# chenzpstar/Multi-Modal-Image-Fusion

Measured on AMD Instinct MI355X. Metric: image-pairs/sec at 256x256, PFNet train step, higher is better.
Workload: dtype bf16; 1 GPU; PFNetv1 train step (fwd + SSIM/pixel/grad losses + bwd + clip + Adam), 256x256 synthetic IR/visible pairs, batch 32 per GPU, bf16 feature maps / fp32 accumulate, random-init weights (seed 0); global_batch=32, parallelism=single

## Files before the change

### multi-modal-image-fusion_amd/csrc/conv_mfma.hip

```cpp
#include "common.hpp"
#include "conv_route.hpp"
#include "wgrad_reduce.hpp"
#define MMIF_STORE_GRAN(p, v) (*reinterpret_cast<uint4*>(p) = (v))
#include <stdlib.h>

namespace mmif {

typedef __attribute__((ext_vector_type(8))) __bf16 bf16x8;
typedef __attribute__((ext_vector_type(4))) __bf16 bf16x4;
typedef __attribute__((ext_vector_type(4))) short s16x4;
typedef __attribute__((ext_vector_type(4))) float f32x4;
#define LDS_PTR(T, p) ((__attribute__((address_space(3))) T*)(p))

constexpr int DT_ROWS_C = DT_ROWS;
__host__ __device__ constexpr int plane_granules(int ks) { return ks == 3 ? 336 : 256; }

__host__ __device__ inline int visit_tap(int i, int ks) { return ks == 3 ? (i % 3) * 3 + i / 3 : i; }

static size_t packed_bytes(int n_out, int n_in, int ks) {
    const int ncb = (n_in + 7) / 8, kk = ks * ks;
    const size_t m16p = (size_t)n_mblocks(n_out) * pick_mf(n_out) * 16;
    size_t kg = 0;
    for (int c0 = 0; c0 < ncb; c0 += CHUNK_CB) {
        const int n = ncb - c0 < CHUNK_CB ? ncb - c0 : CHUNK_CB;
        kg += (size_t)((kk * n + 3) / 4) * 4;
    }
    return kg * m16p * 16;
}

__global__ void pack_weights_kernel(const float* __restrict__ w, int cout, int cin, int ks, int dgrad, int mf,
                                    int m16p, bf16_t* __restrict__ dst, long long total) {
    const int kk = ks * ks;
    const int n_out = dgrad ? cin : cout, n_in = dgrad ? cout : cin;
    const int ncb = (n_in + 7) / 8;
    for (long long idx = (long long)blockIdx.x * blockDim.x + threadIdx.x; idx < total; idx += (long long)gridDim.x * blockDim.x) {
        const int e = idx & 7;
        const long long row = idx >> 3;
        const int oc = (int)(row % m16p);
        long long kgp = row / m16p;
        int c0 = 0, n = 0, kg = 0;
        for (c0 = 0; c0 < ncb; c0 += CHUNK_CB) {
            n = ncb - c0 < CHUNK_CB ? ncb - c0 : CHUNK_CB;
            const int pad = ((kk * n + 3) / 4) * 4;
            if (kgp < pad) { kg = (int)kgp; break; }
            kgp -= pad;
        }
        float val = 0.f;
        if (kg < kk * n) {
            const int tap = kg / n, cb = kg % n;
            const int u = tap / ks, v = tap % ks;
            const int ic = (c0 + cb) * 8 + e;
            if (oc < n_out && ic < n_in) {
                if (dgrad) val = w[(((long long)ic * cin + oc) * ks + (ks - 1 - u)) * ks + (ks - 1 - v)];
                else val = w[(((long long)oc * cin + ic) * ks + u) * ks + v];
            }
        }
        dst[idx] = f32_to_bf16(val);
    }
    (void)mf;
}

constexpr int PACK_MAX_IMAGES = 64;
struct PackImage { const float* w; bf16_t* dst; long long total; int cout, cin, ks, dgrad, m16p; };
struct PackTable { PackImage im[PACK_MAX_IMAGES]; };

__device__ inline void pack_gran(const PackImage& J, long long row) {
    const int ks = J.ks, kk = ks * ks, cin = J.cin, m16p = J.m16p;
    const int n_out = J.dgrad ? cin : J.cout, n_in = J.dgrad ? J.cout : cin;
    const int ncb = (n_in + 7) / 8;
    const int oc = (int)(row % m16p);
    long long kgp = row / m16p;
    int c0 = 0, n = 0, kg = 0;
    for (c0 = 0; c0 < ncb; c0 += CHUNK_CB) {
        n = ncb - c0 < CHUNK_CB ? ncb - c0 : CHUNK_CB;
        const int pad = ((kk * n + 3) / 4) * 4;
        if (kgp < pad) { kg = (int)kgp; break; }
        kgp -= pad;
    }
    float val[8];
#pragma unroll
    for (int e = 0; e < 8; ++e) val[e] = 0.f;
    if (kg < kk * n && oc < n_out) {
        const int tap = kg / n, cb = kg % n;
        const int u = tap / ks, v = tap % ks;
        const int ic0 = (c0 + cb) * 8;
#pragma unroll
        for (int e = 0; e < 8; ++e) {
            const int ic = ic0 + e;
            if (ic < n_in) {
                if (J.dgrad) val[e] = J.w[(((long long)ic * cin + oc) * ks + (ks - 1 - u)) * ks + (ks - 1 - v)];
                else val[e] = J.w[(((long long)oc * cin + ic) * ks + u) * ks + v];
            }
        }
    }
    *reinterpret_cast<uint4*>(J.dst + row * 8) = make_uint4(pack_bf16x2(val[0], val[1]), pack_bf16x2(val[2], val[3]), pack_bf16x2(val[4], val[5]), pack_bf16x2(val[6], val[7]));
}

__global__ void pack_weights_multi_kernel(PackTable tab) {
    const PackImage& J = tab.im[blockIdx.y];
    const long long rows = J.total >> 3;
    for (long long row = (long long)blockIdx.x * blockDim.x + threadIdx.x; row < rows; row += (long long)gridDim.x * blockDim.x)
        pack_gran(J, row);
}

__device__ inline uint4 ld_gran(const TV& t, int in_, int c, int ys, int xs) {
    return *reinterpret_cast<const uint4*>(t.base + t.gidx(in_, c, ys, xs) * 16);
}
__device__ inline uint4 load_in_reflect(const TV& t, int in_, int c, int y, int x) {
    y = min(max(reflect_idx(y, t.h), 0), t.h - 1);
    x = min(max(reflect_idx(x, t.w), 0), t.w - 1);
    return ld_gran(t, in_, c, y, x);
}
__device__ inline uint4 load_in_gradfold(const TV& t, int in_, int c, int y, int x) {
    if (y < 0 || y >= t.h || x < 0 || x >= t.w) return make_uint4(0, 0, 0, 0);
    if (t.halo == 0 || t.folded) return ld_gran(t, in_, c, y + t.halo, x + t.halo);
    const bool by = (y == 1) || (y == t.h - 2), bx = (x == 1) || (x == t.w - 2);
    if (!by && !bx) return ld_gran(t, in_, c, y + 1, x + 1);
    float v[8];
    load_grad_fold<bf16_t>(t, in_, c, y, x, v);
    return make_uint4(pack_bf16x2(v[0], v[1]), pack_bf16x2(v[2], v[3]), pack_bf16x2(v[4], v[5]), pack_bf16x2(v[6], v[7]));
}

struct DupOut {
    TV out, mask;
    int frag;
};

template <int MF, bool DGRAD, bool LM = false, bool DUP = false>
__device__ inline void conv_epilogue(const f32x4 (&acc)[MF][4], const TV& tout, const TV& tmask, const float* s_bias, int mb, int in_,
                                     int oxs, int oys0, int g, int relu, unsigned long long mask_bits, unsigned long long accum_bits,
                                     int xlim, int ylim,
                                     const unsigned char* lmask = nullptr, int lrow0 = 0, int lcol = 0,
                                     const TV* told = nullptr ,
                                     const DupOut* dup = nullptr ) {
    if (oxs >= xlim) return;
    const unsigned row_bytes = (unsigned)tout.ws * 16u;
    const unsigned pix_off = (unsigned)(oys0 * tout.ws + oxs) * 16u;
    uint4 oldv[(DGRAD && !DUP) ? MF : 1][2], xmv[(DGRAD && !LM && !DUP) ? MF : 1][2];
    unsigned lbits[(DGRAD && LM) ? MF : 1][2];
    if (DGRAD && LM) {
#pragma unroll
        for (int m = 0; m < MF; ++m)
#pragma unroll
            for (int p2 = 0; p2 < 2; ++p2) lbits[LM ? m : 0][p2] = lmask[((2 * m + (g >> 1)) * DT_ROWS_C + lrow0 + 2 * p2) * MT + lcol];
    }
    if (DGRAD && !DUP) {
        const unsigned mpix_off = (unsigned)min(max(reflect_idx(oxs - tout.halo, tmask.w), 0), tmask.w - 1) * 16u;
#pragma unroll
        for (int m = 0; m < MF; ++m) {
            const int ocb = (mb * MF + m) * 2 + (g >> 1);
            const bool blk_ok = ocb < tout.cb;
            const char* oplane = tout.base + ((long long)in_ * tout.img + (long long)(tout.cb_off + min(ocb, tout.cb - 1)) * tout.plane) * 16 + pix_off;
            if (told != nullptr)
                oplane = told->base + ((long long)in_ * told->img + (long long)(told->cb_off + min(ocb, told->cb - 1)) * told->plane) * 16 +
// ... 240 lines not shown
        } else {
            const bool inside = y >= 0 && y < tin.h && x >= 0 && x < tin.w;
            const bool border = tin.halo && !tin.folded && ((y == 1) || (y == tin.h - 2) || (x == 1) || (x == tin.w - 2));
            mode = !inside ? 0 : (border ? 2 : 1);
            ioff[i] = (unsigned)((min(max(y, 0), tin.h - 1) + tin.halo) * tin.ws + min(max(x, 0), tin.w - 1) + tin.halo) * 16u;
        }
        idesc[i] = (cb * PL + p) | (cb << 16) | (mode << 20);
        ioff[i] += (unsigned)min(cb, CHUNK_CB - 1) * (unsigned)(tin.plane * 16);
    }
    const char* in_img = tin.base + ((long long)in_ * tin.img + (long long)tin.cb_off * tin.plane) * 16;
    const bool fold_tile = DGRAD && tin.halo && !tin.folded &&
                           ((iy0 <= 1 && 1 < iy0 + TP) || (iy0 <= tin.h - 2 && tin.h - 2 < iy0 + TP) ||
                            (ix0 <= 1 && 1 < ix0 + TP) || (ix0 <= tin.w - 2 && tin.w - 2 < ix0 + TP));

    f32x4 acc[MF][4];
#pragma unroll
    for (int m = 0; m < MF; ++m)
#pragma unroll
        for (int n = 0; n < 4; ++n) acc[m][n] = (f32x4){0.f, 0.f, 0.f, 0.f};

    const int ncb_tot = tin.cb;
    const char* in_lane = reinterpret_cast<const char*>(s_in) + ((wave * 4) * TP + j) * 16;
    const char* w_lane = reinterpret_cast<const char*>(s_w) + j * 16;

    constexpr bool WREG = (256 % (MF * 16)) == 0;
    constexpr int NWO = WREG ? 1 : NW;
    unsigned woff[NWO];
#pragma unroll
    for (int i = 0; i < NWO; ++i) {
        const int e = tid + 256 * i;
        woff[i] = (unsigned)((e / (MF * 16)) * m16p + mb * MF * 16 + e % (MF * 16)) * 16u;
    }
    const unsigned wstride = (unsigned)(256 / (MF * 16)) * (unsigned)m16p * 16u;
    uint4 rin[NIN], rw[NW];
    auto issue_load = [&](int i, int c0, long long wchunk_off) {
        const int ncb = min(CHUNK_CB, ncb_tot - c0);
        if (i < NIN) {
            const int cb = (idesc[i] >> 16) & 15, mode = idesc[i] >> 20;
            const char* chunk = in_img + (long long)c0 * tin.plane * 16;
            const uint4 v = *reinterpret_cast<const uint4*>(chunk + (cb < ncb ? ioff[i] : ioff[0]));
            rin[i] = (cb < ncb && mode >= 1) ? v : make_uint4(0, 0, 0, 0);
        } else if (i < NIN + NW) {
            const int nkgp = (KK * ncb + 3) / 4 * 4;
            const char* wchunk = reinterpret_cast<const char*>(wpk + wchunk_off);
            const int e = tid + 256 * (i - NIN);
            uint4 v = make_uint4(0, 0, 0, 0);
            if (e / (MF * 16) < nkgp) {
                if (WREG) v = *reinterpret_cast<const uint4*>(wchunk + (long long)(i - NIN) * wstride + woff[0]);
                else v = *reinterpret_cast<const uint4*>(wchunk + woff[WREG ? 0 : i - NIN]);
            }
            rw[i - NIN] = v;
        }
    };
    auto prefetch = [&](int c0, long long wchunk_off) {
#pragma unroll
        for (int i = 0; i < NIN + NW; ++i) issue_load(i, c0, wchunk_off);
    };
    if (!DGRAD && tid < MF * 16) {
        const int oc = mb * MF * 16 + tid;
        s_bias[tid] = (bias != nullptr && oc < n_out) ? bias[oc] : 0.f;
    }

    long long wchunk_off = 0;
    TRACE_STAMP();
    prefetch(0, 0);
    TRACE_STAMP();
    for (int c0 = 0; c0 < ncb_tot; c0 += CHUNK_CB) {
        const int ncb = min(CHUNK_CB, ncb_tot - c0);
        const int nkg = KK * ncb, nkgp = (nkg + 3) / 4 * 4;
        __syncthreads();
        TRACE_STAMP();
#pragma unroll
        for (int i = 0; i < NIN; ++i)
            if (((idesc[i] >> 16) & 15) < ncb) s_in[idesc[i] & 0xffff] = rin[i];
        if (DGRAD && fold_tile) {
#pragma unroll 1
            for (int e = tid; e < ncb * TP * TP; e += 256) {
                const int cb = e / (TP * TP), p = e % (TP * TP);
                const int y = iy0 + p / TP, x = ix0 + p % TP;
                const bool inside = y >= 0 && y < tin.h && x >= 0 && x < tin.w;
                if (inside && ((y == 1) || (y == tin.h - 2) || (x == 1) || (x == tin.w - 2)))
                    s_in[cb * PL + p] = load_in_gradfold(tin, in_, c0 + cb, y, x);
            }
        }
#pragma unroll
        for (int i = 0; i < NW; ++i) {
            const int e = tid + 256 * i;
            if (e < nkgp * MF * 16) s_w[e] = rw[i];
        }
        if (tid < nkgp) {
            int tap = 0, cb = 0, plane = tid;
            if (tid < nkg) { tap = visit_tap(tid / ncb, KS); cb = tid % ncb; plane = tap * ncb + cb; }
            s_tab[tid] = make_int2((cb * PL + (tap / KS) * TP + (tap % KS)) * 16, plane * MF * 256);
        }
        TRACE_STAMP();
        __syncthreads();
        TRACE_STAMP();
        wchunk_off += (long long)nkgp * m16p;
        const bool have_next = c0 + CHUNK_CB < ncb_tot;
        const int nsteps = nkgp >> 2;
        if (have_next) prefetch(c0 + CHUNK_CB, wchunk_off);
        int2 off = s_tab[g];
        int2 nxt = s_tab[min(4, nkgp - 4) + g];
        bf16x8 b[4];
#pragma unroll
        for (int n = 0; n < 4; ++n) b[n] = *reinterpret_cast<const bf16x8*>(in_lane + off.x + n * TP * 16);
        for (int s = 0; s < nsteps; ++s) {
            const int2 nxt2 = s_tab[min(4 * (s + 2), nkgp - 4) + g];
            bf16x8 a[MF], bn[4];
#pragma unroll
            for (int m = 0; m < MF; ++m) a[m] = *reinterpret_cast<const bf16x8*>(w_lane + off.y + m * 256);
#pragma unroll
            for (int n = 0; n < 4; ++n) bn[n] = *reinterpret_cast<const bf16x8*>(in_lane + nxt.x + n * TP * 16);
#pragma unroll
            for (int m = 0; m < MF; ++m)
#pragma unroll
                for (int n = 0; n < 4; ++n) acc[m][n] = __builtin_amdgcn_mfma_f32_16x16x32_bf16(a[m], b[n], acc[m][n], 0, 0, 0);
#pragma unroll
            for (int n = 0; n < 4; ++n) b[n] = bn[n];
            off = nxt;
            nxt = nxt2;
        }
        TRACE_STAMP();
    }

    conv_epilogue<MF, DGRAD>(acc, tout, tmask, s_bias, mb, in_, tile_x * MT + j, tile_y * MT + wave * 4 + (g & 1), g, relu, mask_bits,
                             accum_bits, tout.ws, tout.hs);
    TRACE_STAMP();
    if (tr != nullptr) tr[63] = tr_n;
#undef TRACE_STAMP
}

constexpr int DTP_Y = DT_ROWS + 2, DTP_X = MT + 2;
constexpr int DPL = 624;
constexpr int DIN_PIECES = CHUNK_CB * DPL / 64;
constexpr int DW_PIECES = 36;
constexpr int D_PIECES = DIN_PIECES + DW_PIECES;
constexpr int DBUF_BYTES = CHUNK_CB * DPL * 16 + DW_PIECES * 64 * 16;
static_assert(CHUNK_CB * DPL % 64 == 0, "input planes must be whole DMA pieces");

#define MMIF_GPTR(p) ((const __attribute__((address_space(1))) void*)(p))
#define MMIF_LPTR(p) ((__attribute__((address_space(3))) void*)(p))

struct DItem { int mb, in_, tile_y, tile_x; };

template <int N> struct IC { static constexpr int value = N; };

template <int MF, int NBUF = (MF == 3 ? 1 : 2)>
__device__ inline void dgrad_fold_steps(f32x4 (&acc)[MF][4], const char* in_c, const char* w_c, int ncb, int pitch, int g, int j, int yl,
                                        int xl, int hs, int ws) {
    const int nb = hs - 4 - yl;
    const int jl = 1 - xl, jr = ws - 4 - xl;
    const bool has_t = yl == 0, has_b = nb >= 0 && nb < 4, has_l = jl >= 0, has_r = jr >= 0 && jr < MT;
    if (!(has_t || has_b || has_l || has_r)) return;
    const bf16x8 zero8 = __builtin_bit_cast(bf16x8, make_uint4(0, 0, 0, 0));
    const bool kz = g >= ncb;
    auto ldb = [&](int brow, int bcol, int jsel) {
        bf16x8 b = *reinterpret_cast<const bf16x8*>(in_c + (brow * pitch + bcol) * 16);
        if (kz || (jsel >= 0 && j != jsel)) b = zero8;
        return b;
    };
    auto lda = [&](int tap, int m) { return *reinterpret_cast<const bf16x8*>(w_c + tap * ncb * (MF * 256) + m * 256); };
    auto at_row = [&](int n, auto&& f) {
        if (n == 0) f(IC<0>()); else if (n == 1) f(IC<1>()); else if (n == 2) f(IC<2>()); else f(IC<3>());
    };
    auto row_steps = [&](auto nc, int tap0, int brow) {
        constexpr int n = decltype(nc)::value;
        bf16x8 b[3], a[3][MF];
#pragma unroll
        for (int v = 0; v < 3; ++v) {
            b[v] = ldb(brow, v, -1);
#pragma unroll
            for (int m = 0; m < MF; ++m) a[v][m] = lda(tap0 + v, m);
        }
#pragma unroll
        for (int v = 0; v < 3; ++v)
#pragma unroll
            for (int m = 0; m < MF; ++m) acc[m][n] = __builtin_amdgcn_mfma_f32_16x16x32_bf16(a[v][m], b[v], acc[m][n], 0, 0, 0);
    };
    auto col_steps = [&](int vcol, int bcol, int jsel) {
        constexpr int NB = NBUF;
        bf16x8 a[NB][MF], b[NB][4];
        auto fetch = [&](int u, int slot) {
#pragma unroll
            for (int m = 0; m < MF; ++m) a[slot][m] = lda(3 * u + vcol, m);
#pragma unroll
            for (int n = 0; n < 4; ++n) b[slot][n] = ldb(n + u, bcol, jsel);
        };
        if (NB == 2) fetch(0, 0);
#pragma unroll
        for (int u = 0; u < 3; ++u) {
            if (NB == 1) fetch(u, 0);
            else if (u + 1 < 3) fetch(u + 1, (u + 1) & 1);
#pragma unroll
            for (int m = 0; m < MF; ++m)
#pragma unroll
                for (int n = 0; n < 4; ++n)
                    acc[m][n] = __builtin_amdgcn_mfma_f32_16x16x32_bf16(a[u & (NB - 1)][m], b[u & (NB - 1)][n], acc[m][n], 0, 0, 0);
        }
    };
    auto corner = [&](auto nc, int tap, int brow, int bcol, int jsel) {
        constexpr int n = decltype(nc)::value;
        const bf16x8 b = ldb(brow, bcol, jsel);
#pragma unroll
        for (int m = 0; m < MF; ++m) acc[m][n] = __builtin_amdgcn_mfma_f32_16x16x32_bf16(lda(tap, m), b, acc[m][n], 0, 0, 0);
    };
    if (has_t) {
        row_steps(IC<1>(), 6, 1);
        if (has_l) corner(IC<1>(), 8, 1, 0, jl);
        if (has_r) corner(IC<1>(), 6, 1, 2, jr);
    }
    if (has_b) {
        at_row(nb, [&](auto nc) {
            constexpr int n = decltype(nc)::value;
            row_steps(nc, 0, n + 2);
            if (has_l) corner(nc, 2, n + 2, 0, jl);
            if (has_r) corner(nc, 0, n + 2, 2, jr);
        });
    }
    if (has_l) col_steps(2, 0, jl);
    if (has_r) col_steps(0, 2, jr);
}

constexpr int D_CONS = 8;
constexpr int D_LOAD = 4;
constexpr int DL_IN_ITERS = (DIN_PIECES + D_LOAD - 1) / D_LOAD;

constexpr int SIGN_XOFF = 15;
struct SignMap {
    unsigned char* p;
    int cb, hs, pitch;
};
static inline int sign_pitch(int w) { return (cdiv(w, MT) + 2) * MT; }

template <bool DIAG> struct DiagArgs {};
template <> struct DiagArgs<true> {
    long long* trace;
    int abl;
};
template <bool DGRAD, int LMASK, bool DUP = false, bool DIAG = false>
__global__ __launch_bounds__((D_CONS + D_LOAD) * 64, 3) void conv_dma_kernel(TV tin, TV tout, TV tmask, const uint4* __restrict__ wpk,
                                                                              const float* __restrict__ bias, int n_out, int m16p, int relu,
                                                                              unsigned long long mask_bits, unsigned long long accum_bits,
                                                                              int tiles_x, int tiles_y, int nmb, int org, SignMap sgn, DupOut dup,
                                                                              DiagArgs<DIAG> diag) {
    constexpr int MF = 4;
    long long* trace = nullptr;
    int abl = 0;
    if constexpr (DIAG) { trace = diag.trace; abl = diag.abl; }
    __shared__ __attribute__((aligned(16))) char s_buf[2 * DBUF_BYTES];
    __shared__ int2 s_tab[2][DW_PIECES];
    __shared__ __attribute__((aligned(16))) float s_bias[3][MF * 16];
    __shared__ __attribute__((aligned(16))) int4 s_item[3];
    __shared__ __attribute__((aligned(16))) unsigned char s_mask[LMASK ? 2 : 1][LMASK ? 8 * DT_ROWS * MT : 16];

    const int tid = threadIdx.x, lane = tid & 63;
    const int wave = __builtin_amdgcn_readfirstlane(tid >> 6);
    const int j = lane & 15, g = lane >> 4;
    int tr_n = 0;
    long long* tr = (trace != nullptr && blockIdx.x < 128 && lane == 0 && wave < D_CONS) ? trace + ((long long)blockIdx.x * 8 + wave) * 64 : nullptr;
#define DTRACE() do { if (tr != nullptr && tr_n < 62 && !(abl & 256)) tr[tr_n++] = (long long)__builtin_amdgcn_s_memtime(); } while (0)
#define DTRACE_TOP(q) do { if (tr != nullptr && tr_n < 62 && (!(abl & 256) || (q) % 3 == 0)) tr[tr_n++] = (long long)__builtin_amdgcn_s_memtime(); } while (0)
    if (tr != nullptr && tr_n < 62) tr[tr_n++] = (long long)__builtin_amdgcn_s_memtime();
    const int tpi = tiles_x * tiles_y;
    const int nitems = tpi * tout.n * nmb;
    int first, stride, count;
    {
        const int G = gridDim.x, b = blockIdx.x;
        if ((G & 7) == 0) {
            const int xcd = b & 7, slot = b >> 3, nsl = G >> 3;
            const int q8 = nitems >> 3, r8 = nitems & 7;
            const int band0 = xcd < r8 ? xcd * (q8 + 1) : r8 * (q8 + 1) + (xcd - r8) * q8;
            const int blen = q8 + (xcd < r8 ? 1 : 0);
            first = band0 + slot;
            stride = nsl;
            count = blen > slot ? (blen - slot + nsl - 1) / nsl : 0;
        } else {
            first = b;
            stride = G;
            count = b < nitems ? (nitems - b + G - 1) / G : 0;
        }
    }
    if (count == 0) return;
    auto decode = [&](int lin) {
        DItem it;
        const unsigned ul = (unsigned)lin, unmb = (unsigned)nmb, utpi = (unsigned)tpi, utx = (unsigned)tiles_x;
        const unsigned tl = ul / unmb;
        it.mb = (int)(ul - tl * unmb);
        const unsigned uin = tl / utpi, trem = tl - uin * utpi;
        const unsigned ty = trem / utx;
        unsigned txx = trem - ty * utx;
        if (org) txx = (txx + ty + uin) % utx;
        it.in_ = (int)uin;
        it.tile_y = (int)ty;
        it.tile_x = (int)txx;
        return it;
    };
    const int ncb_tot = tin.cb;
    const int nch = (ncb_tot + CHUNK_CB - 1) / CHUNK_CB;
    const int ncb_last = ncb_tot - (nch - 1) * CHUNK_CB;
    const int total_q = count * nch;
    if (tid < DW_PIECES) {
        const int kg = tid;
        int tap = 0, cb = 0, plane = kg;
        if (kg < 9 * ncb_last) { tap = visit_tap(kg / ncb_last, 3); cb = kg % ncb_last; plane = tap * ncb_last + cb; }
        s_tab[1][kg] = make_int2((cb * DPL + (tap / 3) * DTP_X + (tap % 3)) * 16, plane * MF * 256);
    }
// ... 42 lines not shown
            char* dst_in = s_buf + buf * DBUF_BYTES + lw * 1024;
            char* dst_w = s_buf + buf * DBUF_BYTES + CHUNK_CB * DPL * 16 + kgf * 1024;
            const char* src_in = tin.base + ((long long)itm.in_ * tin.img + (long long)(tin.cb_off + c * CHUNK_CB) * tin.plane) * 16;
            const char* src_w = reinterpret_cast<const char*>(wpk) + ((long long)c * DW_PIECES * m16p + itm.mb * MF * 16) * 16;
            auto pieces = [&](auto full_c) {
                constexpr bool FULL = decltype(full_c)::value != 0;
                if (!skip_in) {
#pragma unroll
                    for (int i = 0; i < DL_IN_ITERS; ++i) {
                        if (i == DL_IN_ITERS - 1 && lw + D_LOAD * i >= DIN_PIECES) break;
                        unsigned off = d_off[i];
                        if (!FULL) {
                            const unsigned cb = (d_cb >> (2 * i)) & 3u;
                            off -= (cb - min(cb, (unsigned)(ncb - 1))) * plane_bytes;
                        }
                        __builtin_amdgcn_global_load_lds(MMIF_GPTR(src_in + off), MMIF_LPTR(dst_in + i * (D_LOAD * 1024)), 16, 0, 0);
                    }
                }
                if (!skip_w) {
                    unsigned woff = w_off0;
                    const int wlim = nkgp - kgf;
#pragma unroll
                    for (int k = 0; k < DW_PIECES / D_LOAD; ++k) {
                        if (FULL || D_LOAD * k < wlim)
                            __builtin_amdgcn_global_load_lds(MMIF_GPTR(src_w + woff), MMIF_LPTR(dst_w + k * (D_LOAD * 1024)), 16, 0, 0);
                        woff += D_LOAD * wstep;
                    }
                }
            };
            if (ncb == CHUNK_CB) pieces(IC<1>());
            else pieces(IC<0>());
        };
        auto load_bias = [&](const DItem& itm, int slot) {
            static_assert(MF * 16 == 64, "the M-block's bias is one wave's worth");
            if (!DGRAD && lw == 0) {
                const int oc = itm.mb * MF * 16 + lane;
                s_bias[slot][lane] = (bias != nullptr && oc < n_out) ? bias[oc] : 0.f;
            }
        };
        uint4 mreg[LMASK == 1 ? 16 : 1];
        bool mpend = false;
        int mpar = 0;
        auto issue_mask = [&](const DItem& itm) {
            const int t = tid - D_CONS * 64;
            if (LMASK == 2) {
                const int cbl = t >> 5, row = t & 31;
                const int ocb = itm.mb * 8 + cbl;
                const bool need = ocb < tout.cb && ((mask_bits >> ocb) & 1ull);
                const int ys = min(org + itm.tile_y * DT_ROWS + row, sgn.hs - 1), xs = org + itm.tile_x * MT;
                mreg[0] = make_uint4(0xffffffffu, 0xffffffffu, 0xffffffffu, 0xffffffffu);
                if (need) mreg[0] = *reinterpret_cast<const uint4*>(sgn.p + (((long long)itm.in_ * sgn.cb + min(ocb, sgn.cb - 1)) * sgn.hs + ys) * sgn.pitch + xs + SIGN_XOFF);
                return;
            }
#pragma unroll
            for (int cbl = 0; cbl < 8; ++cbl) {
                const int ocb = itm.mb * 8 + cbl;
                const bool need = ocb < tout.cb && ((mask_bits >> ocb) & 1ull);
#pragma unroll
                for (int k = 0; k < 2; ++k) {
                    const int p = t + 256 * k, row = p >> 4, col = p & 15;
                    const int oys = org + itm.tile_y * DT_ROWS + row, oxs = org + itm.tile_x * MT + col;
                    const int y = min(max(reflect_idx(oys - tout.halo, tmask.h), 0), tmask.h - 1);
                    const int x = min(max(reflect_idx(oxs - tout.halo, tmask.w), 0), tmask.w - 1);
                    if (need) mreg[LMASK == 1 ? 2 * cbl + k : 0] = *reinterpret_cast<const uint4*>(tmask.base + tmask.gidx(itm.in_, min(ocb, tmask.cb - 1), y, x) * 16);
                }
            }
        };
        auto park_mask = [&](const DItem& itm, int par) {
            const int t = tid - D_CONS * 64;
            if (LMASK == 2) {
                *reinterpret_cast<uint4*>(&s_mask[LMASK ? par : 0][LMASK ? t * MT : 0]) = mreg[0];
                return;
            }
#pragma unroll
            for (int cbl = 0; cbl < 8; ++cbl) {
                const int ocb = itm.mb * 8 + cbl;
                const bool need = ocb < tout.cb && ((mask_bits >> ocb) & 1ull);
                if (!need) continue;
#pragma unroll
                for (int k = 0; k < 2; ++k) {
                    const uint4 v = mreg[LMASK == 1 ? 2 * cbl + k : 0];
                    const uint32_t wv[4] = {v.x, v.y, v.z, v.w};
                    unsigned bits = 0;
#pragma unroll
                    for (int i = 0; i < 4; ++i) {
                        bits |= ((short)(wv[i] & 0xffffu) > 0 ? 1u : 0u) << (2 * i);
                        bits |= ((short)(wv[i] >> 16) > 0 ? 1u : 0u) << (2 * i + 1);
                    }
                    s_mask[LMASK ? par : 0][LMASK ? cbl * (DT_ROWS * MT) + t + 256 * k : 0] = (unsigned char)bits;
                }
            }
        };
        auto publish = [&](const DItem& itm, int slot) {
            if (lw == 0) {
                s_item[slot] = make_int4(itm.mb, itm.in_, itm.tile_y, itm.tile_x);
                __asm__ volatile("s_waitcnt lgkmcnt(0)" ::: "memory");
            }
        };
        DItem cur = decode(first), mitem = cur;
        publish(cur, 0);
        make_desc(cur);
        load_bias(cur, 0);
        issue_dma(cur, 0, 0);
        int c = 0, item_i = 0;
        if (LMASK && nch == 2) { issue_mask(cur); mitem = cur; mpar = 0; mpend = true; }
        for (int q = 0; q < total_q; ++q) {
            __builtin_amdgcn_s_waitcnt(0x0f70);
            __builtin_amdgcn_s_barrier();
            if (LMASK && mpend) {
                park_mask(mitem, mpar);
                __asm__ volatile("s_waitcnt lgkmcnt(0)" ::: "memory");
                mpend = false;
            }
            if (++c == nch) {
                c = 0;
                ++item_i;
                if (q + 1 < total_q) {
                    cur = decode(first + item_i * stride);
                    publish(cur, item_i % 3);
                    make_desc(cur);
                    load_bias(cur, item_i % 3);
                }
            }
            if (q + 1 < total_q && !(abl & 1)) issue_dma(cur, c, (q & 1) ^ 1, item_i);
            if (LMASK && q + 1 < total_q && c == nch - 2) { issue_mask(cur); mitem = cur; mpar = item_i & 1; mpend = true; }
        }
        return;
    }

    f32x4 acc[MF][4];
#define DMA_EPILOGUE(itm, slot, par)                                                                                                          \
    do {                                                                                                                                      \
        const int oxs_ = org + (itm).tile_x * MT + j, oys0_ = org + (itm).tile_y * DT_ROWS + wave * 4 + (g & 1);                              \
        if constexpr (!DGRAD) {                                                                                                               \
            conv_epilogue_packed<MF, false>(acc, tout, s_bias[slot], (itm).mb, (itm).in_, org + (itm).tile_x * MT,                            \
                                            org + (itm).tile_y * DT_ROWS + wave * 4, wave * 4, relu, mask_bits, tout.ws - org, tout.hs - org,  \
                                            nullptr, tr, &tr_n);                                                                                     \
        } else if constexpr (LMASK != 0) {                                                                                                    \
            if (accum_bits == 0)                                                                                                              \
                conv_epilogue_packed<MF, true>(acc, tout, s_bias[slot], (itm).mb, (itm).in_, org + (itm).tile_x * MT,                         \
                                               org + (itm).tile_y * DT_ROWS + wave * 4, wave * 4, relu, mask_bits, tout.ws - org,             \
                                               tout.hs - org, s_mask[LMASK ? (par) : 0]);                                                     \
            else                                                                                                                              \
                conv_epilogue<MF, true, true>(acc, tout, tmask, s_bias[slot], (itm).mb, (itm).in_, oxs_, oys0_, g, relu, mask_bits,           \
                                              accum_bits, tout.ws - org, tout.hs - org, s_mask[LMASK ? (par) : 0], wave * 4 + (g & 1), j);    \
        } else {                                                                                                                              \
            conv_epilogue<MF, true, false, DUP>(acc, tout, tmask, s_bias[slot], (itm).mb, (itm).in_, oxs_, oys0_, g, relu, mask_bits,        \
                                                accum_bits, tout.ws - org, tout.hs - org, nullptr, wave * 4 + (g & 1), j, nullptr, &dup);     \
        }                                                                                                                                     \
    } while (0)
    DItem cur = {0, 0, 0, 0}, pend = cur;
    bool have_pend = false;
    int pend_slot = 0, pend_par = 0;
    int c = 0, item_i = 0;
    for (int q = 0; q < total_q; ++q) {
        const int buf = q & 1;
        DTRACE_TOP(q);
        __builtin_amdgcn_s_barrier();
        DTRACE();
        int lane_q;
        __asm__ volatile("v_mbcnt_lo_u32_b32 %0, -1, 0\n\tv_mbcnt_hi_u32_b32 %0, -1, %0" : "=v"(lane_q));
        const int j = lane_q & 15, g = lane_q >> 4;
        if (c == 0) {
            const int4 it4 = s_item[item_i % 3];
            cur.mb = __builtin_amdgcn_readfirstlane(it4.x);
            cur.in_ = __builtin_amdgcn_readfirstlane(it4.y);
            cur.tile_y = __builtin_amdgcn_readfirstlane(it4.z);
            cur.tile_x = __builtin_amdgcn_readfirstlane(it4.w);
        }
        if (have_pend) {
            __builtin_amdgcn_s_setprio(3);
            DMA_EPILOGUE(pend, pend_slot, pend_par);
            __builtin_amdgcn_s_setprio(0);
            have_pend = false;
        }
        DTRACE();
        const int ncb = min(CHUNK_CB, ncb_tot - c * CHUNK_CB);
        const char* in_lane = s_buf + buf * DBUF_BYTES + ((wave * 4) * DTP_X + j) * 16;
        const char* w_lane = s_buf + buf * DBUF_BYTES + CHUNK_CB * DPL * 16 + j * 16;
        const bool rows_live = !DGRAD || org + cur.tile_y * DT_ROWS + wave * 4 < tout.hs - org;
        if (c == 0) {
#pragma unroll
            for (int m = 0; m < MF; ++m)
#pragma unroll
                for (int n = 0; n < 4; ++n) acc[m][n] = (f32x4){0.f, 0.f, 0.f, 0.f};
        }
        if (!rows_live) {
        } else if (ncb == CHUNK_CB) {
            const char* in_g = in_lane + g * (DPL * 16);
            const char* w_g = w_lane + g * (MF * 256);
            bf16x8 a[2][MF], rows[8];
            auto ld_row = [&](int v, int r) { return *reinterpret_cast<const bf16x8*>(in_g + (r * DTP_X + v) * 16); };
            auto ld_a = [&](int t, int slot) {
                const int tap = (t % 3) * 3 + t / 3;
#pragma unroll
                for (int m = 0; m < MF; ++m) a[slot][m] = *reinterpret_cast<const bf16x8*>(w_g + tap * 4 * MF * 256 + m * 256);
            };
#pragma unroll
            for (int r = 0; r < 4; ++r) rows[r] = ld_row(0, r);
            ld_a(0, 0);
#pragma unroll
            for (int t = 0; t < 9; ++t) {
                const int v = t / 3, u = t % 3;
                int nreads = 0;
                if (t + 1 < 9) {
                    const int v1 = (t + 1) / 3, u1 = (t + 1) % 3;
                    if (u1 == 0) {
#pragma unroll
                        for (int r = 0; r < 4; ++r) rows[(6 * v1 + r) % 8] = ld_row(v1, r);
                        nreads += 4;
                    } else {
                        rows[(6 * v1 + 3 + u1) % 8] = ld_row(v1, 3 + u1);
                        nreads += 1;
                    }
                    ld_a(t + 1, (t + 1) & 1);
                    nreads += MF;
                }
#pragma unroll
                for (int m = 0; m < MF; ++m)
#pragma unroll
                    for (int n = 0; n < 4; ++n)
                        acc[m][n] = __builtin_amdgcn_mfma_f32_16x16x32_bf16(a[t & 1][m], rows[(6 * v + u + n) % 8], acc[m][n], 0, 0, 0);
                if (t + 1 < 9) {
#pragma unroll
                    for (int r = 0; r < 5; ++r) {
                        __builtin_amdgcn_sched_group_barrier(0x100, 1, 0);
                        __builtin_amdgcn_sched_group_barrier(0x008, 1, 0);
                    }
                    if ((t + 1) % 3 == 0) {
#pragma unroll
                        for (int r = 0; r < 3; ++r) {
                            __builtin_amdgcn_sched_group_barrier(0x100, 1, 0);
                            __builtin_amdgcn_sched_group_barrier(0x008, 1, 0);
                        }
                        __builtin_amdgcn_sched_group_barrier(0x008, 8, 0);
                    } else {
                        __builtin_amdgcn_sched_group_barrier(0x008, 11, 0);
                    }
                }
                (void)nreads;
            }
        } else {
            const int nkgp = (9 * ncb + 3) / 4 * 4, nsteps = nkgp >> 2;
            const int2* tab = s_tab[1];
            int2 off = tab[g];
            int2 nx = tab[min(4, nkgp - 4) + g];
            bf16x8 b[4];
#pragma unroll
            for (int n = 0; n < 4; ++n) b[n] = *reinterpret_cast<const bf16x8*>(in_lane + off.x + n * DTP_X * 16);
            for (int s2 = 0; s2 < nsteps; ++s2) {
                const int2 nx2 = tab[min(4 * (s2 + 2), nkgp - 4) + g];
                bf16x8 a[MF], bn[4];
#pragma unroll
                for (int m = 0; m < MF; ++m) a[m] = *reinterpret_cast<const bf16x8*>(w_lane + off.y + m * 256);
#pragma unroll
                for (int n = 0; n < 4; ++n) bn[n] = *reinterpret_cast<const bf16x8*>(in_lane + nx.x + n * DTP_X * 16);
#pragma unroll
                for (int m = 0; m < MF; ++m)
#pragma unroll
                    for (int n = 0; n < 4; ++n) acc[m][n] = __builtin_amdgcn_mfma_f32_16x16x32_bf16(a[m], b[n], acc[m][n], 0, 0, 0);
#pragma unroll
                for (int n = 0; n < 4; ++n) b[n] = bn[n];
                off = nx;
                nx = nx2;
            }
        }
        if (DGRAD && org && rows_live && !(abl & 4))
            dgrad_fold_steps<MF>(acc, in_lane + min(g, ncb - 1) * (DPL * 16), w_lane + min(g, ncb - 1) * (MF * 256), ncb, DTP_X, g, j,
                                 cur.tile_y * DT_ROWS + wave * 4, cur.tile_x * MT, tout.hs, tout.ws);
        DTRACE();
        if (++c == nch) {
            c = 0;
            if (wave < 4) {
                DMA_EPILOGUE(cur, item_i % 3, item_i & 1);
            } else {
                pend = cur;
                pend_slot = item_i % 3;
                pend_par = item_i & 1;
                have_pend = true;
            }
            ++item_i;
        }
        DTRACE();
    }
    if (tr != nullptr) { tr[63] = tr_n; tr[62] = (long long)__builtin_amdgcn_s_memtime(); }
#undef DTRACE
#undef DTRACE_TOP
    if (have_pend) DMA_EPILOGUE(pend, pend_slot, pend_par);
#undef DMA_EPILOGUE
}


__device__ inline void tn_wait_vmcnt(int n) {
    switch (n) {
        case 0: __builtin_amdgcn_s_waitcnt(0x0f70); break;
        case 1: __builtin_amdgcn_s_waitcnt(0x0f71); break;
        case 2: __builtin_amdgcn_s_waitcnt(0x0f72); break;
        case 3: __builtin_amdgcn_s_waitcnt(0x0f73); break;
        case 4: __builtin_amdgcn_s_waitcnt(0x0f74); break;
        case 5: __builtin_amdgcn_s_waitcnt(0x0f75); break;
        case 6: __builtin_amdgcn_s_waitcnt(0x0f76); break;
        case 7: __builtin_amdgcn_s_waitcnt(0x0f77); break;
        case 8: __builtin_amdgcn_s_waitcnt(0x0f78); break;
        case 9: __builtin_amdgcn_s_waitcnt(0x0f79); break;
        case 10: __builtin_amdgcn_s_waitcnt(0x0f7a); break;
        case 11: __builtin_amdgcn_s_waitcnt(0x0f7b); break;
        case 12: __builtin_amdgcn_s_waitcnt(0x0f7c); break;
        case 13: __builtin_amdgcn_s_waitcnt(0x0f7d); break;
        case 14: __builtin_amdgcn_s_waitcnt(0x0f7e); break;
        case 15: __builtin_amdgcn_s_waitcnt(0x0f7f); break;
        default: __builtin_amdgcn_s_waitcnt(0x4f70); break;
    }
}
__device__ inline void tn_wait_counter(volatile unsigned* ctr, unsigned target) {
    const unsigned a = (unsigned)(size_t)ctr;
    for (int spin = 0; spin < (1 << 22); ++spin) {
        unsigned v;
        __asm__ volatile("ds_read_b32 %0, %1\n\ts_waitcnt lgkmcnt(0)" : "=v"(v) : "v"(a) : "memory");
        if (v >= target) break;
        __builtin_amdgcn_s_sleep(1);
    }
    __asm__ volatile("" ::: "memory");
}

template <int MF, bool DGRAD, int GROUPS = TN_GROUPS, int PL = TN_PL, int MAXP = 8, int RING = tn_ring_bytes(MF), bool TIGHT = false>
__global__ __launch_bounds__((4 * GROUPS + TN_LOAD) * 64, GROUPS == TN_GROUPS ? 4 : 3) void thin_conv_async_kernel(
    TV tin, TV tout, TV tmask, const uint4* __restrict__ wpk, const float* __restrict__ bias, int n_out, int relu,
    unsigned long long mask_bits, unsigned long long accum_bits, int tiles_x, int tiles_y, int ntiles, int org, TV told, int use_old) {
    constexpr int TP = MT + 2;
    constexpr int NCONS = 4 * GROUPS;
    __shared__ __attribute__((aligned(16))) char s_in[RING];
    __shared__ __attribute__((aligned(16))) uint4 s_w[TN_MAXKG * MF * 16];
    __shared__ int2 s_tab[2][36];
    __shared__ __attribute__((aligned(16))) float s_bias[MF * 16];
    __shared__ unsigned s_ready[TN_MAXSLOTS], s_done[TN_MAXSLOTS];
    const int tid = threadIdx.x, lane = tid & 63;
    const int wave = __builtin_amdgcn_readfirstlane(tid >> 6);
    const int j = lane & 15, g = lane >> 4;
    const int G = gridDim.x, b = blockIdx.x;
    const int tpi = tiles_x * tiles_y;
    const int ncb_tot = tin.cb;
    const int nch = (ncb_tot + CHUNK_CB - 1) / CHUNK_CB;
    const int nmine = b < ntiles ? (ntiles - b + G - 1) / G : 0;
    if (nmine == 0) return;
    auto tile_of = [&](int i, int& in_, int& tile_y, int& tile_x) {
        int lin = i;
        if ((G & 7) == 0) {
            const int q8 = ntiles >> 3, r8 = ntiles & 7, xcd = i & 7;
            lin = (xcd < r8 ? xcd * (q8 + 1) : r8 * (q8 + 1) + (xcd - r8) * q8) + (i >> 3);
        }
        in_ = lin / tpi;
        const int trem = lin - in_ * tpi;
        tile_y = trem / tiles_x;
        tile_x = trem - tile_y * tiles_x;
        if (org) tile_x = (tile_x + tile_y + in_) % tiles_x;
    };
    const int in_pieces = (ncb_tot * PL + 63) / 64;
    const int P = (in_pieces + TN_LOAD - 1) / TN_LOAD;
    const int slot_bytes = TIGHT ? in_pieces * 1024 : P * TN_LOAD * 1024;
    const int NS = min(TN_MAXSLOTS, RING / slot_bytes);
    const int D = min(2, NS - GROUPS);

    if (tid < 72) {
        const int c = tid / 36, kg = tid % 36;
        const int ncb = min(CHUNK_CB, ncb_tot - c * CHUNK_CB);
        if (ncb > 0) {
            int tap = 0, cb = 0, plane = kg;
            if (kg < 9 * ncb) { tap = visit_tap(kg / ncb, 3); cb = kg % ncb; plane = tap * ncb + cb; }
            s_tab[c][kg] = make_int2(((c * CHUNK_CB + cb) * PL + (tap / 3) * TP + (tap % 3)) * 16, (c * 36 + plane) * MF * 256);
        }
    }
    if (!DGRAD && tid < MF * 16) s_bias[tid] = (bias != nullptr && tid < n_out) ? bias[tid] : 0.f;
    if (tid < TN_MAXSLOTS) { s_ready[tid] = 0u; s_done[tid] = 0u; }
    if (wave >= NCONS) {
        int wbytes = 0;
        for (int c = 0; c < nch; ++c) wbytes += ((9 * min(CHUNK_CB, ncb_tot - c * CHUNK_CB) + 3) / 4 * 4) * MF * 256;
        const char* src = reinterpret_cast<const char*>(wpk) + lane * 16;
        char* dst = reinterpret_cast<char*>(s_w);
        for (int pz = wave - NCONS; pz * 1024 < wbytes; pz += TN_LOAD)
            __builtin_amdgcn_global_load_lds(MMIF_GPTR(src + (long long)pz * 1024), MMIF_LPTR(dst + pz * 1024), 16, 0, 0);
        __builtin_amdgcn_s_waitcnt(0x0f70);
    }
    __syncthreads();

    if (wave >= NCONS) {
        const int lw = wave - NCONS;
        unsigned geo[MAXP];
#pragma unroll
        for (int i = 0; i < MAXP; ++i) {
            const int slot = min(min(lw + TN_LOAD * i, in_pieces - 1) * 64 + lane, ncb_tot * PL - 1);
            const int pl = slot / PL, p = min(slot - pl * PL, TP * TP - 1);
            geo[i] = (unsigned)(pl << 16 | (p / TP) << 8 | (p % TP));
        }
        const unsigned plane_bytes = (unsigned)(tin.plane * 16);
        auto issue_tile = [&](int k) {
            int in_, ty0, tx0;
            tile_of(b + k * G, in_, ty0, tx0);
            const int iy0 = ty0 * MT - tout.halo - 1 + org, ix0 = tx0 * MT - tout.halo - 1 + org;
            const char* src = tin.base + ((long long)in_ * tin.img + (long long)tin.cb_off * tin.plane) * 16;
            char* dst = s_in + (k % NS) * slot_bytes;
#pragma unroll
            for (int i = 0; i < MAXP; ++i) {
                if (i < P) {
                    const int piece = min(lw + TN_LOAD * i, in_pieces - 1);
                    const int pl = (int)(geo[i] >> 16);
                    int y = iy0 + (int)((geo[i] >> 8) & 255u), x = ix0 + (int)(geo[i] & 255u);
                    if (!DGRAD) {
                        y = min(max(reflect_idx(y, tin.h), 0), tin.h - 1);
                        x = min(max(reflect_idx(x, tin.w), 0), tin.w - 1);
                    } else {
                        y = min(max(y + 1, 0), tin.hs - 1);
                        x = min(max(x + 1, 0), tin.ws - 1);
                    }
                    const unsigned off = (unsigned)(y * tin.ws + x) * 16u + (unsigned)pl * plane_bytes;
                    __builtin_amdgcn_global_load_lds(MMIF_GPTR(src + off), MMIF_LPTR(dst + piece * 1024), 16, 0, 0);
                }
            }
        };
        auto publish = [&](int k) {
            if (lane == 0) {
                const unsigned a = (unsigned)(size_t)&s_ready[k % NS], one = 1u;
                __asm__ volatile("ds_add_u32 %0, %1" : : "v"(a), "v"(one) : "memory");
// ... 1264 lines not shown
```

Baseline: 9292 image-pairs/s.

## Issue chunk barrier early inside the last MFMA tap for upper waves

Waves 4 and up can now execute the per-chunk workgroup barrier before the final tap of the 9-tap MFMA loop, once their LDS reads have drained, and then skip the barrier at the top of the next iteration. This overlaps barrier waiting with the last MFMA batch so double-buffered DMA can advance sooner. It is restricted to full chunks, live rows, no dgrad border folding, and dgrad with at least three chunks, because other paths may still read the buffer after the barrier. The barrier counts per wave must match exactly, or the block can hang or race on LDS.

```diff
diff --git a/multi-modal-image-fusion_amd/csrc/chunk_skew.hpp b/multi-modal-image-fusion_amd/csrc/chunk_skew.hpp
--- /dev/null
+++ b/multi-modal-image-fusion_amd/csrc/chunk_skew.hpp
@@ -0,0 +1,33 @@
+#pragma once
+
+#if defined(__HIPCC__) || defined(__CUDACC__)
+#define MMIF_SKEW_HD __host__ __device__
+#else
+#define MMIF_SKEW_HD
+#endif
+
+#ifndef MMIF_SKEW_FIRST_WAVE
+#define MMIF_SKEW_FIRST_WAVE 4
+#endif
+#ifndef MMIF_SKEW_DGRAD_MIN_NCH
+#define MMIF_SKEW_DGRAD_MIN_NCH 3
+#endif
+
+namespace mmif {
+
+MMIF_SKEW_HD inline bool dgrad_fold_any(int yl, int xl, int hs, int ws, int mt) {
+    const int nb = hs - 4 - yl, jl = 1 - xl, jr = ws - 4 - xl;
+    return yl == 0 || (nb >= 0 && nb < 4) || jl >= 0 || (jr >= 0 && jr < mt);
+}
+
+MMIF_SKEW_HD inline bool chunk_barrier_early(bool dgrad, int wave, int q, int total_q, int c, int nch, bool last_full, bool rows_live, bool folds) {
+    if (wave < MMIF_SKEW_FIRST_WAVE) return false;
+    if (dgrad && nch < MMIF_SKEW_DGRAD_MIN_NCH) return false;
+    if (q + 1 >= total_q) return false;
+    const bool cur_full = last_full || c != nch - 1;
+    const int c1 = c + 1 == nch ? 0 : c + 1;
+    const bool next_full = last_full || c1 != nch - 1;
+    return cur_full && next_full && rows_live && !folds;
+}
+
+}
diff --git a/multi-modal-image-fusion_amd/csrc/conv_mfma.hip b/multi-modal-image-fusion_amd/csrc/conv_mfma.hip
--- a/multi-modal-image-fusion_amd/csrc/conv_mfma.hip
+++ b/multi-modal-image-fusion_amd/csrc/conv_mfma.hip
@@ -1,5 +1,6 @@
 #include "common.hpp"
 #include "conv_route.hpp"
+#include "chunk_skew.hpp"
 #include "wgrad_reduce.hpp"
 #define MMIF_STORE_GRAN(p, v) (*reinterpret_cast<uint4*>(p) = (v))
 #include <stdlib.h>
@@ -546,7 +547,7 @@
     const int nb = hs - 4 - yl;
     const int jl = 1 - xl, jr = ws - 4 - xl;
     const bool has_t = yl == 0, has_b = nb >= 0 && nb < 4, has_l = jl >= 0, has_r = jr >= 0 && jr < MT;
-    if (!(has_t || has_b || has_l || has_r)) return;
+    if (!dgrad_fold_any(yl, xl, hs, ws, MT)) return;
     const bf16x8 zero8 = __builtin_bit_cast(bf16x8, make_uint4(0, 0, 0, 0));
     const bool kz = g >= ncb;
     auto ldb = [&](int brow, int bcol, int jsel) {
@@ -895,11 +896,13 @@
     DItem cur = {0, 0, 0, 0}, pend = cur;
     bool have_pend = false;
     int pend_slot = 0, pend_par = 0;
+    bool early = false;
+    const bool last_full = ncb_last == CHUNK_CB;
     int c = 0, item_i = 0;
     for (int q = 0; q < total_q; ++q) {
         const int buf = q & 1;
         DTRACE_TOP(q);
-        __builtin_amdgcn_s_barrier();
+        if (!early) __builtin_amdgcn_s_barrier();
         DTRACE();
         int lane_q;
         __asm__ volatile("v_mbcnt_lo_u32_b32 %0, -1, 0\n\tv_mbcnt_hi_u32_b32 %0, -1, %0" : "=v"(lane_q));
@@ -922,6 +925,9 @@
         const char* in_lane = s_buf + buf * DBUF_BYTES + ((wave * 4) * DTP_X + j) * 16;
         const char* w_lane = s_buf + buf * DBUF_BYTES + CHUNK_CB * DPL * 16 + j * 16;
         const bool rows_live = !DGRAD || org + cur.tile_y * DT_ROWS + wave * 4 < tout.hs - org;
+        bool folds = false;
+        if constexpr (DGRAD) folds = org && dgrad_fold_any(cur.tile_y * DT_ROWS + wave * 4, cur.tile_x * MT, tout.hs, tout.ws, MT);
+        const bool go = chunk_barrier_early(DGRAD, wave, q, total_q, c, nch, last_full, rows_live, folds);
         if (c == 0) {
 #pragma unroll
             for (int m = 0; m < MF; ++m)
@@ -942,9 +948,20 @@
 #pragma unroll
             for (int r = 0; r < 4; ++r) rows[r] = ld_row(0, r);
             ld_a(0, 0);
+            if constexpr (DIAG) {
+                if (abl & 512) {
+                    __asm__ volatile("s_waitcnt lgkmcnt(0)" ::: "memory");
+                    DTRACE();
+                }
+            }
 #pragma unroll
             for (int t = 0; t < 9; ++t) {
                 const int v = t / 3, u = t % 3;
+                if (t == 8 && go) {
+                    __builtin_amdgcn_sched_barrier(0);
+                    __asm__ volatile("s_waitcnt lgkmcnt(0)\n\ts_barrier" ::: "memory");
+                    __builtin_amdgcn_sched_barrier(0);
+                }
                 int nreads = 0;
                 if (t + 1 < 9) {
                     const int v1 = (t + 1) / 3, u1 = (t + 1) % 3;
@@ -1011,6 +1028,7 @@
         if (DGRAD && org && rows_live && !(abl & 4))
             dgrad_fold_steps<MF>(acc, in_lane + min(g, ncb - 1) * (DPL * 16), w_lane + min(g, ncb - 1) * (MF * 256), ncb, DTP_X, g, j,
                                  cur.tile_y * DT_ROWS + wave * 4, cur.tile_x * MT, tout.hs, tout.ws);
+        early = go;
         DTRACE();
         if (++c == nch) {
             c = 0;
```

Result: no change. 9330 image-pairs/s, median of 6 (+0.4%).
